# tahmidawal/Superresolution_for_PDEs

Hardware: AMD Instinct MI355X
Metric: 20->40 SR training samples/sec at batch 1024 per GPU (fwd+MSE bwd+clip+AdamW) (higher is better)
Workload: dtype f32 (h3: fp32 products from power-of-two-scaled 2-piece fp16 splits on fp16 MFMA, fp32 accumulate); 1 GPU; UNet 20->40 train step, fp32, batch 1024/GPU, 40x40; global_batch=1024, per_gpu_batch=1024, hw=40x40, parallelism=dp1

## Files before the change

### superresolution_for_pdes_amd/csrc/pointwise.hip

```cpp
#include "bn_reduce.h"

namespace srpde {

__global__ void nchw_to_nhwc_kernel(const float* __restrict__ x, float* __restrict__ out, int N, int Cin, int HW,
                                    int Cpad) {
  const long long total = (long long)N * HW;
  for (long long e = blockIdx.x * (long long)blockDim.x + threadIdx.x; e < total;
       e += (long long)gridDim.x * blockDim.x) {
    const long long n = e / HW;
    const int p = (int)(e - n * HW);
    float* o = out + e * Cpad;
    for (int c = 0; c < Cpad; ++c) o[c] = c < Cin ? x[(n * Cin + c) * HW + p] : 0.f;
  }
}

__global__ void nhwc_to_nchw_kernel(const float* __restrict__ x, int ldx, float* __restrict__ out, int N, int C,
                                    int HW) {
  const long long total = (long long)N * C * HW;
  for (long long e = blockIdx.x * (long long)blockDim.x + threadIdx.x; e < total;
       e += (long long)gridDim.x * blockDim.x) {
    const long long nc = e / HW;
    const int p = (int)(e - nc * HW);
    const long long n = nc / C;
    const int c = (int)(nc - n * C);
// ... 522 lines not shown
  }
  __syncthreads();
  for (int j = threadIdx.x; j < C; j += blockDim.x) m[(long long)n * C + j] = ms[j];
  for (int r = threadIdx.x; r < Cr; r += blockDim.x) {
    float a = b1[r];
    for (int c = 0; c < C; ++c) a += w1[r * C + c] * ms[c];
    a = fmaxf(a, 0.f);
    hs[r] = a;
    h[(long long)n * Cr + r] = a;
  }
  __syncthreads();
  for (int c = threadIdx.x; c < C; c += blockDim.x) {
    float a = b2[c];
    for (int r = 0; r < Cr; ++r) a += w2[c * Cr + r] * hs[r];
    ca[(long long)n * C + c] = 1.f / (1.f + expf(-a));
  }
}

__global__ __launch_bounds__(256) void att_spatial_fwd_kernel(const float* __restrict__ g, int ldg, long long P,
                                                              int G, const float* __restrict__ wg,
                                                              const float* __restrict__ bg, float* __restrict__ sa) {
  const int sub = threadIdx.x & 7;
  for (long long p = (blockIdx.x * (long long)blockDim.x + threadIdx.x) >> 3; p < P;
       p += ((long long)gridDim.x * blockDim.x) >> 3) {
    float acc = 0.f;
    const float* row = g + p * ldg;
    for (int c = sub * 4; c < G; c += 32) {
      const float4 v = ld4(row + c);
      const float4 w = ld4(wg + c);
      acc += dot4(v, w);
    }
    acc += __shfl_xor(acc, 1, 64);
    acc += __shfl_xor(acc, 2, 64);
    acc += __shfl_xor(acc, 4, 64);
    if (sub == 0) sa[p] = 1.f / (1.f + expf(-(acc + bg[0])));
  }
}

__global__ void att_apply_kernel(const float* __restrict__ x, int ldx, const float* __restrict__ ca,
                                 const float* __restrict__ sa, float* __restrict__ out, int ldo, long long P, int HW,
                                 int C) {
  const int C4 = C >> 2;
  const long long total = P * C4;
  for (long long e = blockIdx.x * (long long)blockDim.x + threadIdx.x; e < total;
       e += (long long)gridDim.x * blockDim.x) {
    const long long p = e / C4;
    const int c = (int)(e - p * C4) * 4;
    const long long n = p / HW;
    const float4 v = ld4(x + p * ldx + c);
    const float4 a = ld4(ca + n * C + c);
    const float s = sa[p];
    float4 o;
    o.x = (v.x * a.x) * s; o.y = (v.y * a.y) * s; o.z = (v.z * a.z) * s; o.w = (v.w * a.w) * s;
    *reinterpret_cast<float4*>(out + p * ldo + c) = o;
  }
}

__global__ __launch_bounds__(256) void att_bwd_pixel_kernel(const float* __restrict__ dout, int lddo,
                                                            const float* __restrict__ x, int ldx,
                                                            const float* __restrict__ ca,
                                                            const float* __restrict__ sa, long long P, int HW, int C,
                                                            float* __restrict__ dsa_pre) {
  const int sub = threadIdx.x & 7;
  for (long long p = (blockIdx.x * (long long)blockDim.x + threadIdx.x) >> 3; p < P;
       p += ((long long)gridDim.x * blockDim.x) >> 3) {
    const long long n = p / HW;
    float acc = 0.f;
    for (int c = sub * 4; c < C; c += 32) {
      const float4 d = ld4(dout + p * lddo + c);
      const float4 v = ld4(x + p * ldx + c);
      const float4 a = ld4(ca + n * C + c);
      acc += d.x * (v.x * a.x) + d.y * (v.y * a.y) + d.z * (v.z * a.z) + d.w * (v.w * a.w);
    }
    acc += __shfl_xor(acc, 1, 64);
    acc += __shfl_xor(acc, 2, 64);
    acc += __shfl_xor(acc, 4, 64);
    if (sub == 0) {
      const float s = sa[p];
      dsa_pre[p] = acc * (1.f - s) * s;
    }
  }
}

__global__ __launch_bounds__(256) void att_bwd_channel_kernel(
    const float* __restrict__ dout, int lddo, const float* __restrict__ x, int ldx, const float* __restrict__ sa,
    int HW, int C, int Cr, const float* __restrict__ w1, const float* __restrict__ w2, const float* __restrict__ m,
    const float* __restrict__ h, const float* __restrict__ ca, float* __restrict__ dm,
    float* __restrict__ dw1_rows, float* __restrict__ db1_rows, float* __restrict__ dw2_rows,
    float* __restrict__ db2_rows) {
  extern __shared__ float sh[];
  const int n = blockIdx.x, C4 = C >> 2;
  const int c4 = threadIdx.x % C4, r0 = threadIdx.x / C4, rs = blockDim.x / C4;
  const int active = C4 * rs;
  float4 s = zero4();
  if ((int)threadIdx.x < active) {
    const long long pb = (long long)n * HW;
    for (int p = r0; p < HW; p += rs) {
      const float4 d = ld4(dout + (pb + p) * lddo + c4 * 4);
      const float4 v = ld4(x + (pb + p) * ldx + c4 * 4);
      const float q = sa[pb + p];
      s.x += (d.x * q) * v.x; s.y += (d.y * q) * v.y; s.z += (d.z * q) * v.z; s.w += (d.w * q) * v.w;
    }
  }
  float4* red = reinterpret_cast<float4*>(sh);
  red[threadIdx.x] = s;
  __syncthreads();
  float* dpre = sh + 4 * 256;
  float* dh = dpre + C;
  if ((int)threadIdx.x < C4) {
    const float4 t = rowsum4(red, C4, rs, threadIdx.x);
    const int c = threadIdx.x * 4;
    const float tv[4] = {t.x, t.y, t.z, t.w};
#pragma unroll
    for (int k = 0; k < 4; ++k) {
      const float a = ca[(long long)n * C + c + k];
      dpre[c + k] = tv[k] * (1.f - a) * a;
    }
  }
  __syncthreads();
  for (int c = threadIdx.x; c < C; c += blockDim.x) db2_rows[(long long)n * C + c] = dpre[c];
  for (int r = threadIdx.x; r < Cr; r += blockDim.x) {
    float a = 0.f;
    for (int c = 0; c < C; ++c) a += w2[c * Cr + r] * dpre[c];
    a = h[(long long)n * Cr + r] > 0.f ? a : 0.f;
    dh[r] = a;
    db1_rows[(long long)n * Cr + r] = a;
  }
  __syncthreads();
  for (int c = threadIdx.x; c < C; c += blockDim.x) {
    float a = 0.f;
    for (int r = 0; r < Cr; ++r) a += w1[r * C + c] * dh[r];
    dm[(long long)n * C + c] = a / (float)HW;
  }
}

__global__ __launch_bounds__(256) void att_bwd_sample_kernel(
    const float* __restrict__ dout, int lddo, const float* __restrict__ x, int ldx, const float* __restrict__ sa,
    int HW, int C, int Cr, const float* __restrict__ w1, const float* __restrict__ w2, const float* __restrict__ m,
    const float* __restrict__ h, const float* __restrict__ ca, float* __restrict__ dm, float* __restrict__ dw1_rows,
    float* __restrict__ db1_rows, float* __restrict__ dw2_rows, float* __restrict__ db2_rows,
    float* __restrict__ dsa_pre) {
  extern __shared__ float sh[];
  const int n = blockIdx.x, C4 = C >> 2;
  const int c4 = threadIdx.x % C4, r0 = threadIdx.x / C4, rs = blockDim.x / C4;
  float4 s = zero4();
  {
    const float4 a = ld4(ca + (long long)n * C + c4 * 4);
    const long long pb = (long long)n * HW;
    for (int p = r0; p < HW; p += rs) {
      const float4 d = ld4(dout + (pb + p) * lddo + c4 * 4);
      const float4 v = ld4(x + (pb + p) * ldx + c4 * 4);
      const float q = sa[pb + p];
      s.x += (d.x * q) * v.x; s.y += (d.y * q) * v.y; s.z += (d.z * q) * v.z; s.w += (d.w * q) * v.w;
      float dot = d.x * (v.x * a.x) + d.y * (v.y * a.y) + d.z * (v.z * a.z) + d.w * (v.w * a.w);
      for (int o = C4 >> 1; o > 0; o >>= 1) dot += __shfl_xor(dot, o, 64);
      if (c4 == 0) dsa_pre[pb + p] = dot * (1.f - q) * q;
    }
  }
  float4* red = reinterpret_cast<float4*>(sh);
  red[threadIdx.x] = s;
  __syncthreads();
  float* dpre = sh + 4 * 256;
  float* dh = dpre + C;
  if ((int)threadIdx.x < C4) {
    const float4 t = rowsum4(red, C4, rs, threadIdx.x);
    const int c = threadIdx.x * 4;
    const float tv[4] = {t.x, t.y, t.z, t.w};
#pragma unroll
    for (int k = 0; k < 4; ++k) {
      const float a = ca[(long long)n * C + c + k];
      dpre[c + k] = tv[k] * (1.f - a) * a;
    }
  }
  __syncthreads();
  for (int c = threadIdx.x; c < C; c += blockDim.x) db2_rows[(long long)n * C + c] = dpre[c];
  for (int r = threadIdx.x; r < Cr; r += blockDim.x) {
    float a = 0.f;
    for (int c = 0; c < C; ++c) a += w2[c * Cr + r] * dpre[c];
    a = h[(long long)n * Cr + r] > 0.f ? a : 0.f;
    dh[r] = a;
    db1_rows[(long long)n * Cr + r] = a;
  }
  __syncthreads();
  for (int c = threadIdx.x; c < C; c += blockDim.x) {
    float a = 0.f;
    for (int r = 0; r < Cr; ++r) a += w1[r * C + c] * dh[r];
    dm[(long long)n * C + c] = a / (float)HW;
  }
}

__global__ void att_bwd_dx_kernel(const float* __restrict__ dout, int lddo, const float* __restrict__ ca,
                                  const float* __restrict__ sa, const float* __restrict__ dm, float* __restrict__ dx,
                                  int lddx, long long P, int HW, int C, int accumulate) {
  const int C4 = C >> 2;
  const long long total = P * C4;
  for (long long e = blockIdx.x * (long long)blockDim.x + threadIdx.x; e < total;
       e += (long long)gridDim.x * blockDim.x) {
    const long long p = e / C4;
    const int c = (int)(e - p * C4) * 4;
    const long long n = p / HW;
    const float4 d = ld4(dout + p * lddo + c);
    const float4 a = ld4(ca + n * C + c);
    const float4 g = ld4(dm + n * C + c);
    const float s = sa[p];
    float4 o = gate_dx4(d, s, a, g);
    float* dst = dx + p * lddx + c;
    if (accumulate) o = add4(o, ld4(dst));
    st4(dst, o);
  }
}

__global__ void att_bwd_gating_kernel(const float* __restrict__ dsa_pre, const float* __restrict__ wg,
                                      float* __restrict__ dg, int lddg, long long P, int G, int accumulate) {
  const int G4 = G >> 2;
  const long long total = P * G4;
  for (long long e = blockIdx.x * (long long)blockDim.x + threadIdx.x; e < total;
       e += (long long)gridDim.x * blockDim.x) {
    const long long p = e / G4;
    const int c = (int)(e - p * G4) * 4;
    const float s = dsa_pre[p];
    const float4 w = ld4(wg + c);
    float4 o = scale4(s, w);
    float* dst = dg + p * lddg + c;
    if (accumulate) o = add4(o, ld4(dst));
    st4(dst, o);
  }
}

__global__ __launch_bounds__(256) void weighted_colsum_kernel(const float* __restrict__ v, int ldv,
                                                              const float* __restrict__ s, long long P, int C,
                                                              int rows_per_blk, float2* __restrict__ part) {
  extern __shared__ float4 red4[];
  const int C4 = C >> 2;
  const int c4 = threadIdx.x % C4, r0 = threadIdx.x / C4, rs = blockDim.x / C4;
  const int active = C4 * rs;
  float4 acc = zero4();
  float sacc = 0.f;
  const long long pb = (long long)blockIdx.x * rows_per_blk;
  const long long pe = min(P, pb + rows_per_blk);
  if ((int)threadIdx.x < active) {
    auto row = [&](const float4& a, float w) {
      acc.x += a.x * w; acc.y += a.y * w; acc.z += a.z * w; acc.w += a.w * w;
      if (c4 == 0) sacc += w;
    };
    long long p = pb + r0;
    for (; p + 3 * rs < pe; p += 4 * rs) {
      float4 a[4];
      float w[4];
#pragma unroll
      for (int u = 0; u < 4; ++u) {
        a[u] = ld4(v + (p + u * rs) * ldv + c4 * 4);
        w[u] = s[p + u * rs];
      }
#pragma unroll
      for (int u = 0; u < 4; ++u) row(a[u], w[u]);
    }
    for (; p < pe; p += rs) row(ld4(v + p * ldv + c4 * 4), s[p]);
  }
  red4[threadIdx.x] = acc;
  red4[256 + threadIdx.x] = make_float4(sacc, 0.f, 0.f, 0.f);
  __syncthreads();
  if ((int)threadIdx.x < C4) {
    float4 t = zero4();
    float ts = 0.f;
    for (int r = 0; r < rs; ++r) {
      const float4 a = red4[r * C4 + threadIdx.x];
      t.x += a.x; t.y += a.y; t.z += a.z; t.w += a.w;
      if (threadIdx.x == 0) ts += red4[256 + r * C4].x;
    }
    float2* o = part + (size_t)blockIdx.x * (C + 1);
    const int c = threadIdx.x * 4;
    o[c] = make_float2(t.x, 0.f); o[c + 1] = make_float2(t.y, 0.f);
    o[c + 2] = make_float2(t.z, 0.f); o[c + 3] = make_float2(t.w, 0.f);
    if (threadIdx.x == 0) o[C] = make_float2(ts, 0.f);
  }
}

__global__ __launch_bounds__(1024) void outer_sum_kernel(const float* __restrict__ a, int la,
                                                         const float* __restrict__ b, int lb, int n,
                                                         float* __restrict__ out) {
  __shared__ double red[16][64];
  const int i = blockIdx.x, jl = threadIdx.x & 63, grp = threadIdx.x >> 6;
  const int j = blockIdx.y * 64 + jl;
  double s = 0.0;
  if (j < lb) {
    int k = grp;
    for (; k + 7 * 16 < n; k += 8 * 16) {
      float av[8], bv[8];
#pragma unroll
      for (int u = 0; u < 8; ++u) {
        av[u] = a ? a[(long long)(k + 16 * u) * la + i] : 1.f;
        bv[u] = b ? b[(long long)(k + 16 * u) * lb + j] : 1.f;
      }
#pragma unroll
      for (int u = 0; u < 8; ++u) s += (double)av[u] * (double)bv[u];
    }
    for (; k < n; k += 16) {
      const double av = a ? (double)a[(long long)k * la + i] : 1.0;
      const double bv = b ? (double)b[(long long)k * lb + j] : 1.0;
      s += av * bv;
    }
  }
  red[grp][jl] = s;
  __syncthreads();
  if (grp == 0 && j < lb) {
    double t = 0.0;
    for (int g = 0; g < 16; ++g) t += red[g][jl];
    out[(long long)i * lb + j] = (float)t;
  }
}

__global__ void rowsum_kernel(const float* __restrict__ rows, int n, int len, float* __restrict__ out, int stride_in,
                              int accumulate) {
  const int j = blockIdx.x * blockDim.x + threadIdx.x;
  if (j >= len) return;
  double s = 0.0;
  for (int k = 0; k < n; ++k) s += rows[(long long)k * stride_in + j];
  out[j] = accumulate ? out[j] + (float)s : (float)s;
}

__global__ void partsum_kernel(const float2* __restrict__ part, int nblk, int len, float* __restrict__ out) {
  const int j = blockIdx.x;
  __shared__ double a[256];
  double s = 0.0;
  for (int k = threadIdx.x; k < nblk; k += 256) s += part[(size_t)k * len + j].x;
  a[threadIdx.x] = s;
  __syncthreads();
  for (int t = 128; t > 0; t >>= 1) {
    if ((int)threadIdx.x < t) a[threadIdx.x] += a[threadIdx.x + t];
    __syncthreads();
  }
  if (threadIdx.x == 0) out[j] = (float)a[0];
}

__global__ void head_fwd_kernel(const float* __restrict__ z, int ldz, int C, const float* __restrict__ wf,
                                const float* __restrict__ bf, const float* __restrict__ xin, int xin_c, int HW,
                                long long P, float* __restrict__ out) {
  for (long long p = blockIdx.x * (long long)blockDim.x + threadIdx.x; p < P; p += (long long)gridDim.x * blockDim.x) {
    float acc = 0.f;
    for (int c = 0; c < C; c += 4) {
      const float4 v = ld4(z + p * ldz + c);
      acc += v.x * wf[c] + v.y * wf[c + 1] + v.z * wf[c + 2] + v.w * wf[c + 3];
    }
    const long long n = p / HW;
    const int q = (int)(p - n * HW);
    out[p] = (acc + bf[0]) + xin[(n * xin_c) * HW + q];
  }
}

__global__ void head_bwd_dz_kernel(const float* __restrict__ dout, const float* __restrict__ wf, int C,
                                   float* __restrict__ dz, int lddz, long long P) {
  const int C4 = C >> 2;
  const long long total = P * C4;
  for (long long e = blockIdx.x * (long long)blockDim.x + threadIdx.x; e < total;
       e += (long long)gridDim.x * blockDim.x) {
    const long long p = e / C4;
    const int c = (int)(e - p * C4) * 4;
    const float d = dout[p];
    *reinterpret_cast<float4*>(dz + p * lddz + c) = make_float4(d * wf[c], d * wf[c + 1], d * wf[c + 2], d * wf[c + 3]);
  }
}

__global__ __launch_bounds__(256) void mse_partial_kernel(const float* __restrict__ y, const float* __restrict__ t,
                                                          long long n, double* __restrict__ part) {
  __shared__ double red[256];
  double s = 0.0;
  for (long long i = blockIdx.x * (long long)blockDim.x + threadIdx.x; i < n; i += (long long)gridDim.x * blockDim.x) {
    const float d = y[i] - t[i];
    s += (double)(d * d);
  }
  red[threadIdx.x] = s;
  __syncthreads();
  for (int k = 128; k > 0; k >>= 1) {
    if ((int)threadIdx.x < k) red[threadIdx.x] += red[threadIdx.x + k];
    __syncthreads();
  }
  if (threadIdx.x == 0) part[blockIdx.x] = red[0];
}

__global__ void mse_final_kernel(const double* __restrict__ part, int nblk, long long n, float* __restrict__ loss) {
  __shared__ double red[256];
  double s = 0.0;
  for (int k = threadIdx.x; k < nblk; k += 256) s += part[k];
  red[threadIdx.x] = s;
  __syncthreads();
  for (int k = 128; k > 0; k >>= 1) {
    if ((int)threadIdx.x < k) red[threadIdx.x] += red[threadIdx.x + k];
    __syncthreads();
  }
  if (threadIdx.x == 0) loss[0] = (float)(red[0] / (double)n);
}

// ... 64 lines not shown
                         int w, int c, int accumulate, hipStream_t stream) {
  SRPDE_CHECK_ARG(x && dout && dx && c % 4 == 0 && h % 2 == 0 && w % 2 == 0, "srpde_maxpool2x2_bwd: bad args");
  launch_px_or_grid_stride(
      (long long)n * (h / 2) * (w / 2), c,
      [&](dim3 g, dim3 b, unsigned npix) {
        hipLaunchKernelGGL(maxpool2_bwd_px_kernel, g, b, 0, stream, x, ldx, dout, lddo, dx, lddx, npix, h, w, accumulate);
      },
      [&](dim3 g) {
        hipLaunchKernelGGL(maxpool2_bwd_kernel, g, dim3(256), 0, stream, x, ldx, dout, lddo, dx, lddx, n, h, w, c,
                           accumulate);
      });
  SRPDE_LAUNCH_CHECK("srpde_maxpool2x2_bwd");
  return 0;
}

int srpde_pde_dataset_assemble(const float* u_coarse, const float* u_fine, const float* theta_fine,
                               const float* f_fine, const float* stats, int theta_constant, int n, int hc, int wc,
                               int hf, int wf, float* inputs, float* targets, hipStream_t stream) {
  SRPDE_CHECK_ARG(u_coarse && u_fine && theta_fine && f_fine && stats && inputs && targets,
                  "srpde_pde_dataset_assemble: null");
  SRPDE_CHECK_ARG(n >= 0 && hc >= 1 && wc >= 1 && hf >= hc && wf >= wc, "srpde_pde_dataset_assemble: bad shape");
  if (n == 0) return 0;
  hipLaunchKernelGGL(pde_dataset_kernel, dim3(grid_for((long long)n * hf * wf)), dim3(256), 0, stream, u_coarse,
                     u_fine, theta_fine, f_fine, stats, theta_constant, n, hc, wc, hf, wf, inputs, targets);
  SRPDE_LAUNCH_CHECK("srpde_pde_dataset_assemble");
  return 0;
}

int srpde_upsample_bilinear_fwd(const float* x, int ldx, float* out, int ldo, int n, int h, int w, int ho, int wo,
                                int c, hipStream_t stream) {
  SRPDE_CHECK_ARG(x && out && c > 0, "srpde_upsample_bilinear_fwd: bad args");
  if (c % 4 != 0 || ldx % 4 != 0 || ldo % 4 != 0) {
    hipLaunchKernelGGL(upsample_fwd_scalar_kernel, dim3(grid_for((long long)n * ho * wo * c)), dim3(256), 0, stream,
                       x, ldx, out, ldo, n, h, w, ho, wo, c);
    SRPDE_LAUNCH_CHECK("srpde_upsample_bilinear_fwd");
    return 0;
  }
  launch_px_or_grid_stride(
      (long long)n * ho * wo, c,
      [&](dim3 g, dim3 b, unsigned npix) {
        hipLaunchKernelGGL(upsample_fwd_px_kernel, g, b, 0, stream, x, ldx, out, ldo, npix, h, w, ho, wo);
      },
      [&](dim3 g) {
        hipLaunchKernelGGL(upsample_fwd_kernel, g, dim3(256), 0, stream, x, ldx, out, ldo, n, h, w, ho, wo, c);
      });
  SRPDE_LAUNCH_CHECK("srpde_upsample_bilinear_fwd");
  return 0;
}

int srpde_upsample_bilinear_gate_fwd(const float* x, int ldx, float* out, int ldo, int n, int h, int w, int ho,
                                      int wo, int c, const float* wg, const float* bg, float* sa, hipStream_t stream) {
  SRPDE_CHECK_ARG(x && out && wg && bg && sa && ldx % 4 == 0 && ldo % 4 == 0 && c % 4 == 0 && c / 4 >= 1 &&
                      c / 4 <= 64 && ((c / 4) & (c / 4 - 1)) == 0,
                  "srpde_upsample_bilinear_gate_fwd: bad args (c / 4 a power of two <= 64)");
  dim3 g, b;
  SRPDE_CHECK_ARG(px_geometry((long long)n * ho * wo, c, &g, &b), "srpde_upsample_bilinear_gate_fwd: bad geometry");
  g.x = (g.x + UPX - 1) / UPX;
  hipLaunchKernelGGL(upsample_gate_fwd_px_kernel, g, b, 0, stream, x, ldx, out, ldo, (unsigned)(n * ho * wo), h, w,
                     ho, wo, wg, bg, sa);
  SRPDE_LAUNCH_CHECK("srpde_upsample_bilinear_gate_fwd");
  return 0;
}

size_t srpde_upsample_gate_sa_workspace_size(int n, int h, int w) { return (size_t)n * h * w * sizeof(float); }

int srpde_upsample_gate_sa(const float* x, int ldx, int n, int h, int w, int ho, int wo, int c, const float* wg,
                           const float* bg, float* sa, void* workspace, size_t ws_bytes, hipStream_t stream) {
  SRPDE_CHECK_ARG(x && wg && bg && sa && workspace && ldx % 4 == 0 && c % 4 == 0 && c / 4 >= 1 && c / 4 <= 64 &&
                      ((c / 4) & (c / 4 - 1)) == 0 && n > 0 && h > 0 && w > 0 && ho > 0 && wo > 0,
                  "srpde_upsample_gate_sa: bad args (c / 4 a power of two <= 64)");
  SRPDE_CHECK_ARG(ws_bytes >= srpde_upsample_gate_sa_workspace_size(n, h, w), "srpde_upsample_gate_sa: workspace");
  float* t = static_cast<float*>(workspace);
  dim3 g, b;
  SRPDE_CHECK_ARG(px_geometry((long long)n * h * w, c, &g, &b), "srpde_upsample_gate_sa: bad geometry");
  hipLaunchKernelGGL(gate_dot_px_kernel, g, b, 0, stream, x, ldx, (unsigned)(n * h * w), wg, t);
  SRPDE_LAUNCH_CHECK("srpde_upsample_gate_sa(dot)");
  const unsigned np = (unsigned)(n * ho * wo);
  hipLaunchKernelGGL(up_sigmoid_kernel, dim3((np + 255) / 256), dim3(256), 0, stream, t, sa, np, h, w, ho, wo, bg);
  SRPDE_LAUNCH_CHECK("srpde_upsample_gate_sa(up)");
  return 0;
}

static size_t att_lds_bytes(int c) { return (4 * 256 + c + c / 8) * sizeof(float); }

static void launch_att_channel(const float* x, int ldx, int n, int hw, int c, const float* w1, const float* b1,
                               const float* w2, const float* b2, float* m, float* hbuf, float* ca, hipStream_t stream) {
  hipLaunchKernelGGL(att_channel_fwd_kernel, dim3(n), dim3(256), att_lds_bytes(c), stream, x, ldx, hw, c, c / 8, w1, b1,
                     w2, b2, m, hbuf, ca);
}
static void launch_att_spatial(const float* g, int ldg, long long P, int gc, const float* wg, const float* bg, float* sa,
                               hipStream_t stream) {
  hipLaunchKernelGGL(att_spatial_fwd_kernel, dim3(grid_for(P * 8)), dim3(256), 0, stream, g, ldg, P, gc, wg, bg, sa);
}
static void launch_att_apply(const float* x, int ldx, const float* ca, const float* sa, float* out, int ldo, long long P,
                             int hw, int c, hipStream_t stream) {
  hipLaunchKernelGGL(att_apply_kernel, dim3(grid_for(P * (c / 4))), dim3(256), 0, stream, x, ldx, ca, sa, out, ldo, P,
                     hw, c);
}

int srpde_att_apply_fwd(const float* x, int ldx, int n, int hw, int c, const float* ca, const float* sa, float* out,
                        int ldo, hipStream_t stream) {
  SRPDE_CHECK_ARG(x && ca && sa && out && c % 4 == 0, "srpde_att_apply_fwd: bad args");
  launch_att_apply(x, ldx, ca, sa, out, ldo, (long long)n * hw, hw, c, stream);
  SRPDE_LAUNCH_CHECK("srpde_att_apply_fwd");
  return 0;
}

int srpde_upsample_bilinear_bwd_gated(const float* dout, int lddo, const float* dsa, const float* wg, float* dx,
                                      int lddx, int n, int h, int w, int ho, int wo, int c, int accumulate,
                                      hipStream_t stream) {
  SRPDE_CHECK_ARG(dout && dsa && wg && dx && c % 4 == 0 && lddo % 4 == 0 && lddx % 4 == 0 && ho >= h && wo >= w,
                  "srpde_upsample_bilinear_bwd_gated: bad args");
  SRPDE_CHECK_ARG(upsample_gather_ok(h, ho) && upsample_gather_ok(w, wo),
                  "srpde_upsample_bilinear_bwd_gated: upsampling ratio above 4 (%dx%d -> %dx%d)", h, w, ho, wo);
  if (upsample_rows_ok(h, w, ho, wo, c, lddo, lddx)) {
    launch_upsample_bwd_rows<true>(dout, lddo, dx, lddx, n, h, w, ho, wo, c, accumulate, dsa, wg, stream);
    SRPDE_LAUNCH_CHECK("srpde_upsample_bilinear_bwd_gated");
    return 0;
  }
  dim3 g, b;
  SRPDE_CHECK_ARG(px_geometry((long long)n * h * w, c, &g, &b),
                  "srpde_upsample_bilinear_bwd_gated: needs c / 4 a power of two <= 256 (c=%d)", c);
  hipLaunchKernelGGL(upsample_bwd_px_kernel, g, b, 0, stream, dout, lddo, dx, lddx, (unsigned)(n * h * w), h, w, ho,
                     wo, accumulate, dsa, wg);
  SRPDE_LAUNCH_CHECK("srpde_upsample_bilinear_bwd_gated");
  return 0;
}

int srpde_upsample_bwd_bn_supported(int h, int w, int ho, int wo, int c, int lddo, int lddx) {
  return upsample_gather_ok(h, ho) && upsample_gather_ok(w, wo) && upsample_rows_ok(h, w, ho, wo, c, lddo, lddx) ? 1
                                                                                                               : 0;
}

int srpde_upsample_bilinear_bwd_gated_bn(const float* dout, int lddo, const float* dsa, const float* wg, float* dx,
                                         int lddx, int n, int h, int w, int ho, int wo, int c, const float* y, int ldy,
                                         const float* mean, const float* invstd, const float* gamma,
                                         const float* beta, int flags, void* part, float* da_max,
                                         hipStream_t stream) {
  SRPDE_CHECK_ARG(dout && dsa && wg && dx && y && mean && invstd && gamma && beta && part && da_max && ldy % 4 == 0 &&
                      aligned16(y) && aligned16(dx) && aligned16(dout),
                  "srpde_upsample_bilinear_bwd_gated_bn: null argument / alignment");
  SRPDE_CHECK_ARG(ho >= h && wo >= w && srpde_upsample_bwd_bn_supported(h, w, ho, wo, c, lddo, lddx),
                  "srpde_upsample_bilinear_bwd_gated_bn: shape outside the row-blocked kernel "
                  "(srpde_upsample_bwd_bn_supported)");
  const UpBnArgs bn{y, ldy, mean, invstd, gamma, beta, flags & SRPDE_BN_RELU, static_cast<float2*>(part), da_max};
  launch_upsample_bwd_rows<true>(dout, lddo, dx, lddx, n, h, w, ho, wo, c, 0, dsa, wg, stream, &bn);
  SRPDE_LAUNCH_CHECK("srpde_upsample_bilinear_bwd_gated_bn");
  return 0;
}

int srpde_upsample_bilinear_bwd(const float* dout, int lddo, float* dx, int lddx, int n, int h, int w, int ho,
                                int wo, int c, int accumulate, hipStream_t stream) {
  SRPDE_CHECK_ARG(dout && dx && c % 4 == 0 && ho >= h && wo >= w, "srpde_upsample_bilinear_bwd: bad args");
  SRPDE_CHECK_ARG(upsample_gather_ok(h, ho) && upsample_gather_ok(w, wo),
                  "srpde_upsample_bilinear_bwd: upsampling ratio above 4 (%dx%d -> %dx%d)", h, w, ho, wo);
  if (upsample_rows_ok(h, w, ho, wo, c, lddo, lddx)) {
    launch_upsample_bwd_rows<false>(dout, lddo, dx, lddx, n, h, w, ho, wo, c, accumulate, nullptr, nullptr, stream);
    SRPDE_LAUNCH_CHECK("srpde_upsample_bilinear_bwd");
    return 0;
  }
  launch_px_or_grid_stride(
      (long long)n * h * w, c,
      [&](dim3 g, dim3 b, unsigned npix) {
        hipLaunchKernelGGL(upsample_bwd_px_kernel, g, b, 0, stream, dout, lddo, dx, lddx, npix, h, w, ho, wo, accumulate);
      },
      [&](dim3 g) {
        hipLaunchKernelGGL(upsample_bwd_kernel, g, dim3(256), 0, stream, dout, lddo, dx, lddx, n, h, w, ho, wo, c,
                           accumulate);
      });
  SRPDE_LAUNCH_CHECK("srpde_upsample_bilinear_bwd");
  return 0;
}

int srpde_att_channel_fwd(const float* x, int ldx, int n, int hw, int c, const float* w1, const float* b1,
                          const float* w2, const float* b2, float* m, float* hbuf, float* ca, hipStream_t stream) {
  SRPDE_CHECK_ARG(x && w1 && b1 && w2 && b2 && m && hbuf && ca, "srpde_att_channel_fwd: null");
  SRPDE_CHECK_ARG(c % 32 == 0 && c <= 1024, "srpde_att_channel_fwd: channel count");
  launch_att_channel(x, ldx, n, hw, c, w1, b1, w2, b2, m, hbuf, ca, stream);
  SRPDE_LAUNCH_CHECK("srpde_att_channel_fwd");
  return 0;
}

int srpde_att_gate_fwd(const float* x, int ldx, const float* g, int ldg, int n, int hw, int c, int gc,
                       const float* ca, const float* wg, const float* bg, float* sa, float* out, int ldo,
                       hipStream_t stream) {
  SRPDE_CHECK_ARG(x && g && ca && wg && bg && sa && out, "srpde_att_gate_fwd: null");
  SRPDE_CHECK_ARG(c % 32 == 0 && gc % 4 == 0 && c <= 1024, "srpde_att_gate_fwd: channel counts");
  const long long P = (long long)n * hw;
  launch_att_spatial(g, ldg, P, gc, wg, bg, sa, stream);
  SRPDE_LAUNCH_CHECK("srpde_att_gate_fwd(spatial)");
  launch_att_apply(x, ldx, ca, sa, out, ldo, P, hw, c, stream);
  SRPDE_LAUNCH_CHECK("srpde_att_gate_fwd(apply)");
  return 0;
}

int srpde_att_fwd(const float* x, int ldx, const float* g, int ldg, int n, int hw, int c, int gc, const float* w1,
                  const float* b1, const float* w2, const float* b2, const float* wg, const float* bg, float* m,
                  float* hbuf, float* ca, float* sa, float* out, int ldo, hipStream_t stream) {
  SRPDE_CHECK_ARG(x && g && w1 && b1 && w2 && b2 && wg && bg && m && hbuf && ca && sa && out,
                  "srpde_att_fwd: null");
  SRPDE_CHECK_ARG(c % 32 == 0 && gc % 4 == 0 && c <= 1024, "srpde_att_fwd: channel counts");
  launch_att_channel(x, ldx, n, hw, c, w1, b1, w2, b2, m, hbuf, ca, stream);
  SRPDE_LAUNCH_CHECK("srpde_att_fwd(channel)");
  const long long P = (long long)n * hw;
  launch_att_spatial(g, ldg, P, gc, wg, bg, sa, stream);
  SRPDE_LAUNCH_CHECK("srpde_att_fwd(spatial)");
  launch_att_apply(x, ldx, ca, sa, out, ldo, P, hw, c, stream);
  SRPDE_LAUNCH_CHECK("srpde_att_fwd(apply)");
  return 0;
}

size_t srpde_att_bwd_workspace_size(int n, int hw, int c, int gc) {
  if (!att_bwd_counts_ok(c, gc)) return 0;
  const long long P = (long long)n * hw;
  const int cr = c / 8;
  int rpb;
  const int nb = colsum_blocks(P, gc, &rpb);
  size_t f = (size_t)P
             + (size_t)n * c
             + (size_t)n * cr * c * 2
             + (size_t)n * (cr + c)
             + (size_t)nb * (gc + 1) * 2;
  return f * sizeof(float) + 256;
}

int srpde_att_bwd(const float* dout, int lddo, const float* x, int ldx, const float* g, int ldg, int n, int hw,
                  int c, int gc, const float* w1, const float* w2, const float* wg, const float* m, const float* hbuf,
                  const float* ca, const float* sa, float* dx, int lddx, int dx_accumulate, float* dg, int lddg,
                  int dg_accumulate, float* dw1, float* db1, float* dw2, float* db2, float* dwg, float* dbg,
                  void* workspace, size_t ws_bytes, hipStream_t stream) {
  SRPDE_CHECK_ARG(dout && x && g && workspace, "srpde_att_bwd: null");
  SRPDE_CHECK_ARG(att_bwd_counts_ok(c, gc), "srpde_att_bwd: channel counts (c %% 32, gc %% 4, both <= 1024)");
  if (ws_bytes < srpde_att_bwd_workspace_size(n, hw, c, gc)) {
    set_error("srpde_att_bwd: workspace too small");
    return kErrWorkspace;
  }
  const long long P = (long long)n * hw;
  const int cr = c / 8;
  float* dsa = static_cast<float*>(workspace);
  float* dm = dsa + P;
  float* dw1r = dm + (size_t)n * c;
  float* dw2r = dw1r + (size_t)n * cr * c;
  float* db1r = dw2r + (size_t)n * cr * c;
  float* db2r = db1r + (size_t)n * cr;
  float2* part = reinterpret_cast<float2*>(db2r + (size_t)n * c + 2);
  part = reinterpret_cast<float2*>((reinterpret_cast<uintptr_t>(part) + 15) & ~uintptr_t(15));

  const size_t lds = att_lds_bytes(c);
  if (c == 64 || c == 128 || c == 256) {
    hipLaunchKernelGGL(att_bwd_sample_kernel, dim3(n), dim3(256), lds, stream, dout, lddo, x, ldx, sa, hw, c, cr, w1,
                       w2, m, hbuf, ca, dm, dw1r, db1r, dw2r, db2r, dsa);
    SRPDE_LAUNCH_CHECK("srpde_att_bwd(sample)");
  } else {
    hipLaunchKernelGGL(att_bwd_pixel_kernel, dim3(grid_for(P * 8)), dim3(256), 0, stream, dout, lddo, x, ldx, ca,
                       sa, P, hw, c, dsa);
    SRPDE_LAUNCH_CHECK("srpde_att_bwd(pixel)");
    hipLaunchKernelGGL(att_bwd_channel_kernel, dim3(n), dim3(256), lds, stream, dout, lddo, x, ldx, sa, hw, c, cr,
                       w1, w2, m, hbuf, ca, dm, dw1r, db1r, dw2r, db2r);
    SRPDE_LAUNCH_CHECK("srpde_att_bwd(channel)");
  }
  if (dx != nullptr) {
    hipLaunchKernelGGL(att_bwd_dx_kernel, dim3(grid_for(P * (c / 4))), dim3(256), 0, stream, dout, lddo, ca, sa, dm,
                       dx, lddx, P, hw, c, dx_accumulate);
    SRPDE_LAUNCH_CHECK("srpde_att_bwd(dx)");
  }
  if (dg != nullptr) {
    hipLaunchKernelGGL(att_bwd_gating_kernel, dim3(grid_for(P * (gc / 4))), dim3(256), 0, stream, dsa, wg, dg, lddg,
                       P, gc, dg_accumulate);
    SRPDE_LAUNCH_CHECK("srpde_att_bwd(gating)");
  }
  if (dw1 == nullptr) return 0;
  return srpde_att_bwd_params(g, ldg, n, hw, c, gc, m, hbuf, dw1, db1, dw2, db2, dwg, dbg, workspace, ws_bytes,
                              stream);
}

__global__ __launch_bounds__(256) void upsample_t_scalar_kernel(const float* __restrict__ dsa, float* __restrict__ st,
                                                                int n, int h, int w, int ho, int wo) {
  const long long q = (long long)blockIdx.x * blockDim.x + threadIdx.x;
  if (q >= (long long)n * h * w) return;
  const int ix = (int)(q % w), iy = (int)((q / w) % h), nn = (int)(q / ((long long)w * h));
  int ylo, yhi, xlo, xhi;
  cand_range(iy, h, ho, &ylo, &yhi);
  cand_range(ix, w, wo, &xlo, &xhi);
  const float* base = dsa + (size_t)nn * ho * wo;
  float s = 0.f;
  for (int oy = ylo; oy <= yhi; ++oy) {
    bool hy;
    const float wy = cand_weight(oy, iy, h, ho, &hy);
    if (!hy) continue;
    float r = 0.f;
    for (int ox = xlo; ox <= xhi; ++ox) {
      bool hx;
      const float wx = cand_weight(ox, ix, w, wo, &hx);
      if (hx) r += wx * base[(size_t)oy * wo + ox];
    }
    s += wy * r;
  }
  st[q] = s;
}

static void att_params_outer(int n, int c, const float* m, const float* hbuf, const float* db1r, const float* db2r,
                             float* dw1, float* db1, float* dw2, float* db2, hipStream_t stream) {
  const int cr = c / 8;
  hipLaunchKernelGGL(outer_sum_kernel, dim3(cr, ceil_div(c, 64)), dim3(1024), 0, stream, db1r, cr, m, c, n, dw1);
  hipLaunchKernelGGL(outer_sum_kernel, dim3(c, ceil_div(cr, 64)), dim3(1024), 0, stream, db2r, c, hbuf, cr, n, dw2);
  hipLaunchKernelGGL(outer_sum_kernel, dim3(1, ceil_div(cr, 64)), dim3(1024), 0, stream, (const float*)nullptr, 1,
                     db1r, cr, n, db1);
  hipLaunchKernelGGL(outer_sum_kernel, dim3(1, ceil_div(c, 64)), dim3(1024), 0, stream, (const float*)nullptr, 1,
                     db2r, c, n, db2);
}

int srpde_att_bwd_params_lowres(const float* d, int ldd, int n, int h, int w, int ho, int wo, int c, int gc,
                                const float* m, const float* hbuf, float* dw1, float* db1, float* dw2, float* db2,
                                float* dwg, float* dbg, void* workspace, size_t ws_bytes, hipStream_t stream) {
  SRPDE_CHECK_ARG(d && m && hbuf && dw1 && db1 && dw2 && db2 && dwg && dbg && workspace && ldd % 4 == 0 && ho >= h &&
                      wo >= w,
                  "srpde_att_bwd_params_lowres: bad args");
  SRPDE_CHECK_ARG(att_bwd_counts_ok(c, gc),
                  "srpde_att_bwd_params_lowres: channel counts (c %% 32, gc %% 4, both <= 1024)");
  const int hw = ho * wo;
  if (ws_bytes < srpde_att_bwd_workspace_size(n, hw, c, gc)) {
    set_error("srpde_att_bwd_params_lowres: workspace too small");
    return kErrWorkspace;
  }
  const long long P = (long long)n * hw, Plo = (long long)n * h * w;
  const int cr = c / 8;
  float* dsa = static_cast<float*>(workspace);
  float* dm = dsa + P;
  float* dw1r = dm + (size_t)n * c;
  float* dw2r = dw1r + (size_t)n * cr * c;
  float* db1r = dw2r + (size_t)n * cr * c;
  float* db2r = db1r + (size_t)n * cr;
  float2* part = reinterpret_cast<float2*>(db2r + (size_t)n * c + 2);
  part = reinterpret_cast<float2*>((reinterpret_cast<uintptr_t>(part) + 15) & ~uintptr_t(15));
  SRPDE_CHECK_ARG(Plo <= 2LL * n * cr * c, "srpde_att_bwd_params_lowres: low-res field larger than its scratch");
  float* st = dw1r;
  att_params_outer(n, c, m, hbuf, db1r, db2r, dw1, db1, dw2, db2, stream);
  SRPDE_LAUNCH_CHECK("srpde_att_bwd_params_lowres(rowsum)");
  hipLaunchKernelGGL(upsample_t_scalar_kernel, dim3((unsigned)((Plo + 255) / 256)), dim3(256), 0, stream, dsa, st, n, h,
                     w, ho, wo);
  SRPDE_LAUNCH_CHECK("srpde_att_bwd_params_lowres(transpose)");
  int rpb;
  const int nb = colsum_blocks(Plo, gc, &rpb);
  hipLaunchKernelGGL(weighted_colsum_kernel, dim3(nb), dim3(256), 2 * 256 * sizeof(float4), stream, d, ldd, st, Plo,
                     gc, rpb, part);
  SRPDE_LAUNCH_CHECK("srpde_att_bwd_params_lowres(colsum)");
  hipLaunchKernelGGL(partsum_kernel, dim3(gc), dim3(256), 0, stream, part, nb, gc + 1, dwg);
  hipLaunchKernelGGL(partsum_kernel, dim3(1), dim3(256), 0, stream, part + gc, nb, gc + 1, dbg);
  SRPDE_LAUNCH_CHECK("srpde_att_bwd_params_lowres(partsum)");
  return 0;
}

int srpde_att_bwd_params(const float* g, int ldg, int n, int hw, int c, int gc, const float* m, const float* hbuf,
                         float* dw1, float* db1, float* dw2, float* db2, float* dwg, float* dbg, void* workspace,
                         size_t ws_bytes, hipStream_t stream) {
  SRPDE_CHECK_ARG(g && m && hbuf && dw1 && db1 && dw2 && db2 && dwg && dbg && workspace,
                  "srpde_att_bwd_params: null");
  SRPDE_CHECK_ARG(att_bwd_counts_ok(c, gc), "srpde_att_bwd_params: channel counts (c %% 32, gc %% 4, both <= 1024)");
  if (ws_bytes < srpde_att_bwd_workspace_size(n, hw, c, gc)) {
    set_error("srpde_att_bwd_params: workspace too small");
    return kErrWorkspace;
  }
  const long long P = (long long)n * hw;
  const int cr = c / 8;
  float* dsa = static_cast<float*>(workspace);
  float* dm = dsa + P;
  float* dw1r = dm + (size_t)n * c;
  float* dw2r = dw1r + (size_t)n * cr * c;
  float* db1r = dw2r + (size_t)n * cr * c;
  float* db2r = db1r + (size_t)n * cr;
  float2* part = reinterpret_cast<float2*>(db2r + (size_t)n * c + 2);
  part = reinterpret_cast<float2*>((reinterpret_cast<uintptr_t>(part) + 15) & ~uintptr_t(15));
  (void)dw1r; (void)dw2r; (void)cr;
  att_params_outer(n, c, m, hbuf, db1r, db2r, dw1, db1, dw2, db2, stream);
  SRPDE_LAUNCH_CHECK("srpde_att_bwd(rowsum)");
  int rpb;
  const int nb = colsum_blocks(P, gc, &rpb);
  hipLaunchKernelGGL(weighted_colsum_kernel, dim3(nb), dim3(256), 2 * 256 * sizeof(float4), stream, g, ldg, dsa, P,
                     gc, rpb, part);
  SRPDE_LAUNCH_CHECK("srpde_att_bwd(colsum)");
  hipLaunchKernelGGL(partsum_kernel, dim3(gc), dim3(256), 0, stream, part, nb, gc + 1, dwg);
  hipLaunchKernelGGL(partsum_kernel, dim3(1), dim3(256), 0, stream, part + gc, nb, gc + 1, dbg);
  SRPDE_LAUNCH_CHECK("srpde_att_bwd(partsum)");
  return 0;
}

int srpde_head_fwd(const float* z, int ldz, int c, const float* wf, const float* bf, const float* xin, int xin_c,
                   int n, int hw, float* out, hipStream_t stream) {
  SRPDE_CHECK_ARG(z && wf && bf && xin && out && c % 4 == 0, "srpde_head_fwd: bad args");
  const long long P = (long long)n * hw;
  hipLaunchKernelGGL(head_fwd_kernel, dim3(grid_for(P)), dim3(256), 0, stream, z, ldz, c, wf, bf, xin, xin_c, hw, P,
                     out);
  SRPDE_LAUNCH_CHECK("srpde_head_fwd");
  return 0;
}

size_t srpde_head_bwd_workspace_size(int n, int hw, int c) {
  if (!colsum_ok(c)) return 0;
  int rpb;
  const int nb = colsum_blocks((long long)n * hw, c, &rpb);
  return (size_t)nb * (c + 1) * sizeof(float2);
}

int srpde_head_bwd(const float* dout, const float* z, int ldz, int c, const float* wf, int n, int hw, float* dz,
                   int lddz, float* dwf, float* dbf, void* workspace, size_t ws_bytes, hipStream_t stream) {
  SRPDE_CHECK_ARG(dout && z && wf && dz && dwf && dbf && workspace, "srpde_head_bwd: bad args");
  SRPDE_CHECK_ARG(colsum_ok(c), "srpde_head_bwd: channel count (c %% 4, 4 <= c <= 1024)");
  if (ws_bytes < srpde_head_bwd_workspace_size(n, hw, c)) {
    set_error("srpde_head_bwd: workspace too small");
    return kErrWorkspace;
  }
  const long long P = (long long)n * hw;
  hipLaunchKernelGGL(head_bwd_dz_kernel, dim3(grid_for(P * (c / 4))), dim3(256), 0, stream, dout, wf, c, dz, lddz, P);
  SRPDE_LAUNCH_CHECK("srpde_head_bwd(dz)");
  int rpb;
  const int nb = colsum_blocks(P, c, &rpb);
  float2* part = static_cast<float2*>(workspace);
  hipLaunchKernelGGL(weighted_colsum_kernel, dim3(nb), dim3(256), 2 * 256 * sizeof(float4), stream, z, ldz, dout, P,
                     c, rpb, part);
  hipLaunchKernelGGL(partsum_kernel, dim3(c), dim3(256), 0, stream, part, nb, c + 1, dwf);
  hipLaunchKernelGGL(partsum_kernel, dim3(1), dim3(256), 0, stream, part + c, nb, c + 1, dbf);
  SRPDE_LAUNCH_CHECK("srpde_head_bwd(reduce)");
  return 0;
}

size_t srpde_mse_workspace_size(void) { return 1024 * sizeof(double); }

int srpde_mse_fwd(const float* y, const float* t, long long n, float* loss, void* workspace, size_t ws_bytes,
                  hipStream_t stream) {
  SRPDE_CHECK_ARG(y && t && loss && workspace && ws_bytes >= 1024 * sizeof(double), "srpde_mse_fwd: bad args");
  const int nb = (int)std::min<long long>(1024, std::max<long long>(1, (n + 255) / 256));
  hipLaunchKernelGGL(mse_partial_kernel, dim3(nb), dim3(256), 0, stream, y, t, n, static_cast<double*>(workspace));
  hipLaunchKernelGGL(mse_final_kernel, dim3(1), dim3(256), 0, stream, static_cast<const double*>(workspace), nb, n,
                     loss);
  SRPDE_LAUNCH_CHECK("srpde_mse_fwd");
  return 0;
}

int srpde_mse_bwd(const float* y, const float* t, long long n, const float* gout, float* dy, hipStream_t stream) {
  SRPDE_CHECK_ARG(y && t && dy, "srpde_mse_bwd: bad args");
  hipLaunchKernelGGL(mse_bwd_kernel, dim3(grid_for(n)), dim3(256), 0, stream, y, t, n, gout, dy);
  SRPDE_LAUNCH_CHECK("srpde_mse_bwd");
  return 0;
}

}
```

Before: 37680 samples/s.

## Tile attention MLP weight-gradient reduction and stage w2 in LDS

Replaces the four outer_sum launches for the attention MLP weight and bias gradients with one tiled kernel. It stages per-sample dh, h, dpre and m slices in LDS and accumulates all four gradients in double, split across sample slices, with a second kernel summing the partials. The backward per-sample kernels now stage w2 into shared memory for the dpre->dh matvec and unroll the pixel loop by four to issue more loads at once. The cost is more LDS per block, which may reduce occupancy, plus an extra partial-sum pass through scratch memory.

Measured after the change: 37810 samples/s (median of 6 runs). Within noise of the previous version (+0.3%).

```diff
diff --git a/superresolution_for_pdes_amd/csrc/pointwise.hip b/superresolution_for_pdes_amd/csrc/pointwise.hip
--- a/superresolution_for_pdes_amd/csrc/pointwise.hip
+++ b/superresolution_for_pdes_amd/csrc/pointwise.hip
@@ -628,6 +628,45 @@
   }
 }
 
+constexpr int kAttW2Stage = 8192;
+
+__device__ __forceinline__ void stage_floats(float* dst, const float* __restrict__ src, int count) {
+  if ((reinterpret_cast<uintptr_t>(src) & 15u) == 0) {
+    for (int i = threadIdx.x * 4; i < count; i += blockDim.x * 4) st4(dst + i, ld4(src + i));
+  } else {
+    for (int i = threadIdx.x; i < count; i += blockDim.x) dst[i] = src[i];
+  }
+}
+
+__device__ __forceinline__ void att_mlp_bwd_tail(const float* dpre, float* dh, float* w2s, int n, int HW, int C, int Cr,
+                                                 const float* __restrict__ w1, const float* __restrict__ w2,
+                                                 const float* __restrict__ h, float* __restrict__ dm,
+                                                 float* __restrict__ db1_rows, float* __restrict__ db2_rows) {
+  for (int c = threadIdx.x; c < C; c += blockDim.x) db2_rows[(long long)n * C + c] = dpre[c];
+  const int r = threadIdx.x;
+  const int rows = min(C, kAttW2Stage / Cr);
+  float a = 0.f;
+  for (int c0 = 0; c0 < C; c0 += rows) {
+    const int nc = min(rows, C - c0);
+    if (c0 > 0) __syncthreads();
+    stage_floats(w2s, w2 + (long long)c0 * Cr, nc * Cr);
+    __syncthreads();
+    if (r < Cr)
+      for (int c = 0; c < nc; ++c) a += w2s[c * Cr + r] * dpre[c0 + c];
+  }
+  if (r < Cr) {
+    a = h[(long long)n * Cr + r] > 0.f ? a : 0.f;
+    dh[r] = a;
+    db1_rows[(long long)n * Cr + r] = a;
+  }
+  __syncthreads();
+  for (int c = threadIdx.x; c < C; c += blockDim.x) {
+    float a = 0.f;
+    for (int r = 0; r < Cr; ++r) a += w1[r * C + c] * dh[r];
+    dm[(long long)n * C + c] = a / (float)HW;
+  }
+}
+
 __global__ __launch_bounds__(256) void att_bwd_channel_kernel(
     const float* __restrict__ dout, int lddo, const float* __restrict__ x, int ldx, const float* __restrict__ sa,
     int HW, int C, int Cr, const float* __restrict__ w1, const float* __restrict__ w2, const float* __restrict__ m,
@@ -664,20 +703,7 @@
     }
   }
   __syncthreads();
-  for (int c = threadIdx.x; c < C; c += blockDim.x) db2_rows[(long long)n * C + c] = dpre[c];
-  for (int r = threadIdx.x; r < Cr; r += blockDim.x) {
-    float a = 0.f;
-    for (int c = 0; c < C; ++c) a += w2[c * Cr + r] * dpre[c];
-    a = h[(long long)n * Cr + r] > 0.f ? a : 0.f;
-    dh[r] = a;
-    db1_rows[(long long)n * Cr + r] = a;
-  }
-  __syncthreads();
-  for (int c = threadIdx.x; c < C; c += blockDim.x) {
-    float a = 0.f;
-    for (int r = 0; r < Cr; ++r) a += w1[r * C + c] * dh[r];
-    dm[(long long)n * C + c] = a / (float)HW;
-  }
+  att_mlp_bwd_tail(dpre, dh, dh + Cr, n, HW, C, Cr, w1, w2, h, dm, db1_rows, db2_rows);
 }
 
 __global__ __launch_bounds__(256) void att_bwd_sample_kernel(
@@ -693,15 +719,27 @@
   {
     const float4 a = ld4(ca + (long long)n * C + c4 * 4);
     const long long pb = (long long)n * HW;
-    for (int p = r0; p < HW; p += rs) {
-      const float4 d = ld4(dout + (pb + p) * lddo + c4 * 4);
-      const float4 v = ld4(x + (pb + p) * ldx + c4 * 4);
-      const float q = sa[pb + p];
+    auto pixel = [&](int p, const float4& d, const float4& v, float q) {
       s.x += (d.x * q) * v.x; s.y += (d.y * q) * v.y; s.z += (d.z * q) * v.z; s.w += (d.w * q) * v.w;
       float dot = d.x * (v.x * a.x) + d.y * (v.y * a.y) + d.z * (v.z * a.z) + d.w * (v.w * a.w);
       for (int o = C4 >> 1; o > 0; o >>= 1) dot += __shfl_xor(dot, o, 64);
       if (c4 == 0) dsa_pre[pb + p] = dot * (1.f - q) * q;
-    }
+    };
+    int p = r0;
+    for (; p + 3 * rs < HW; p += 4 * rs) {
+      float4 d[4], v[4];
+      float q[4];
+#pragma unroll
+      for (int u = 0; u < 4; ++u) {
+        d[u] = ld4(dout + (pb + p + u * rs) * lddo + c4 * 4);
+        v[u] = ld4(x + (pb + p + u * rs) * ldx + c4 * 4);
+        q[u] = sa[pb + p + u * rs];
+      }
+#pragma unroll
+      for (int u = 0; u < 4; ++u) pixel(p + u * rs, d[u], v[u], q[u]);
+    }
+    for (; p < HW; p += rs)
+      pixel(p, ld4(dout + (pb + p) * lddo + c4 * 4), ld4(x + (pb + p) * ldx + c4 * 4), sa[pb + p]);
   }
   float4* red = reinterpret_cast<float4*>(sh);
   red[threadIdx.x] = s;
@@ -719,20 +757,7 @@
     }
   }
   __syncthreads();
-  for (int c = threadIdx.x; c < C; c += blockDim.x) db2_rows[(long long)n * C + c] = dpre[c];
-  for (int r = threadIdx.x; r < Cr; r += blockDim.x) {
-    float a = 0.f;
-    for (int c = 0; c < C; ++c) a += w2[c * Cr + r] * dpre[c];
-    a = h[(long long)n * Cr + r] > 0.f ? a : 0.f;
-    dh[r] = a;
-    db1_rows[(long long)n * Cr + r] = a;
-  }
-  __syncthreads();
-  for (int c = threadIdx.x; c < C; c += blockDim.x) {
-    float a = 0.f;
-    for (int r = 0; r < Cr; ++r) a += w1[r * C + c] * dh[r];
-    dm[(long long)n * C + c] = a / (float)HW;
-  }
+  att_mlp_bwd_tail(dpre, dh, dh + Cr, n, HW, C, Cr, w1, w2, h, dm, db1_rows, db2_rows);
 }
 
 __global__ void att_bwd_dx_kernel(const float* __restrict__ dout, int lddo, const float* __restrict__ ca,
@@ -822,38 +847,125 @@
   }
 }
 
-__global__ __launch_bounds__(1024) void outer_sum_kernel(const float* __restrict__ a, int la,
-                                                         const float* __restrict__ b, int lb, int n,
-                                                         float* __restrict__ out) {
-  __shared__ double red[16][64];
-  const int i = blockIdx.x, jl = threadIdx.x & 63, grp = threadIdx.x >> 6;
-  const int j = blockIdx.y * 64 + jl;
+constexpr int kAttParSamples = 32;
+constexpr int kAttParCols = 32;
+
+template <int NR>
+__global__ __launch_bounds__(256) void att_params_kernel(const float* __restrict__ dh, const float* __restrict__ dpre,
+                                                         const float* __restrict__ m, const float* __restrict__ h,
+                                                         int n, int C, int Cr, int per_slice,
+                                                         double* __restrict__ part, float* __restrict__ dw1,
+                                                         float* __restrict__ db1, float* __restrict__ dw2,
+                                                         float* __restrict__ db2) {
+  constexpr int SB = kAttParSamples, CB = kAttParCols;
+  extern __shared__ float sh[];
+  float* sdh = sh;
+  float* shh = sdh + SB * Cr;
+  float* sdp = shh + SB * Cr;
+  float* sm = sdp + SB * CB;
+  const int t = threadIdx.x, j = t & (CB - 1), rg = t / CB;
+  const int col0 = blockIdx.y * CB;
+  const int kb = blockIdx.x * per_slice, ke = min(n, kb + per_slice);
+  int r1[NR], c2[NR], r2[NR];
+  double a1[NR], a2[NR], s1[NR], s2 = 0.0;
+#pragma unroll
+  for (int i = 0; i < NR; ++i) {
+    r1[i] = min(rg + 8 * i, Cr - 1);
+    const int f = min(t + 256 * i, CB * Cr - 1);
+    c2[i] = f / Cr;
+    r2[i] = f - c2[i] * Cr;
+    a1[i] = a2[i] = s1[i] = 0.0;
+  }
+  const bool al = ((reinterpret_cast<uintptr_t>(dh) | reinterpret_cast<uintptr_t>(dpre) |
+                    reinterpret_cast<uintptr_t>(m) | reinterpret_cast<uintptr_t>(h)) & 15u) == 0;
+  for (int k0 = kb; k0 < ke; k0 += SB) {
+    const int ns = min(SB, ke - k0), nq = ns * Cr;
+    if (k0 > kb) __syncthreads();
+    if (al) {
+      const int ks = t >> 3, q = (t & 7) * 4;
+      float4 p4 = zero4(), m4 = zero4();
+      if (ks < ns) {
+        p4 = ld4(dpre + (long long)(k0 + ks) * C + col0 + q);
+        m4 = ld4(m + (long long)(k0 + ks) * C + col0 + q);
+      }
+      for (int i = t * 4; i < nq; i += 1024) {
+        const float4 x0 = ld4(dh + (long long)k0 * Cr + i);
+        const float4 x1 = ld4(h + (long long)k0 * Cr + i);
+        st4(sdh + i, x0);
+        st4(shh + i, x1);
+      }
+      if (ks < ns) {
+        st4(sdp + ks * CB + q, p4);
+        st4(sm + ks * CB + q, m4);
+      }
+    } else {
+      for (int i = t; i < ns * CB; i += 256) {
+        const long long g = (long long)(k0 + i / CB) * C + col0 + (i & (CB - 1));
+        sdp[i] = dpre[g];
+        sm[i] = m[g];
+      }
+      for (int i = t; i < nq; i += 256) {
+        sdh[i] = dh[(long long)k0 * Cr + i];
+        shh[i] = h[(long long)k0 * Cr + i];
+      }
+    }
+    __syncthreads();
+    for (int k = 0; k < ns; ++k) {
+      const double mv = (double)sm[k * CB + j], pv = (double)sdp[k * CB + j];
+      s2 += pv;
+#pragma unroll
+      for (int i = 0; i < NR; ++i) {
+        const double dv = (double)sdh[k * Cr + r1[i]];
+        a1[i] += dv * mv;
+        s1[i] += dv;
+        a2[i] += (double)sdp[k * CB + c2[i]] * (double)shh[k * Cr + r2[i]];
+      }
+    }
+  }
+  const int W = Cr * C;
+  double* P = part ? part + (size_t)blockIdx.x * (2 * W + Cr + C) : nullptr;
+#pragma unroll
+  for (int i = 0; i < NR; ++i) {
+    const int r = rg + 8 * i, f = t + 256 * i;
+    if (r < Cr) {
+      const int e = r * C + col0 + j;
+      if (P) P[e] = a1[i];
+      else dw1[e] = (float)a1[i];
+      if (j == 0 && blockIdx.y == 0) {
+        if (P) P[2 * W + r] = s1[i];
+        else db1[r] = (float)s1[i];
+      }
+    }
+    if (f < CB * Cr) {
+      const int e = col0 * Cr + f;
+      if (P) P[W + e] = a2[i];
+      else dw2[e] = (float)a2[i];
+    }
+  }
+  if (rg == 0) {
+    if (P) P[2 * W + Cr + col0 + j] = s2;
+    else db2[col0 + j] = (float)s2;
+  }
+}
+
+__global__ __launch_bounds__(256) void att_params_sum_kernel(const double* __restrict__ part, int slices, int C, int Cr,
+                                                             float* __restrict__ dw1, float* __restrict__ db1,
+                                                             float* __restrict__ dw2, float* __restrict__ db2) {
+  const int W = Cr * C, E = 2 * W + Cr + C;
+  const int e = blockIdx.x * 256 + threadIdx.x;
+  if (e >= E) return;
   double s = 0.0;
-  if (j < lb) {
-    int k = grp;
-    for (; k + 7 * 16 < n; k += 8 * 16) {
-      float av[8], bv[8];
-#pragma unroll
-      for (int u = 0; u < 8; ++u) {
-        av[u] = a ? a[(long long)(k + 16 * u) * la + i] : 1.f;
-        bv[u] = b ? b[(long long)(k + 16 * u) * lb + j] : 1.f;
-      }
-#pragma unroll
-      for (int u = 0; u < 8; ++u) s += (double)av[u] * (double)bv[u];
-    }
-    for (; k < n; k += 16) {
-      const double av = a ? (double)a[(long long)k * la + i] : 1.0;
-      const double bv = b ? (double)b[(long long)k * lb + j] : 1.0;
-      s += av * bv;
-    }
-  }
-  red[grp][jl] = s;
-  __syncthreads();
-  if (grp == 0 && j < lb) {
-    double t = 0.0;
-    for (int g = 0; g < 16; ++g) t += red[g][jl];
-    out[(long long)i * lb + j] = (float)t;
-  }
+  int k = 0;
+  for (; k + 7 < slices; k += 8) {
+    double v[8];
+#pragma unroll
+    for (int u = 0; u < 8; ++u) v[u] = part[(size_t)(k + u) * E + e];
+#pragma unroll
+    for (int u = 0; u < 8; ++u) s += v[u];
+  }
+  for (; k < slices; ++k) s += part[(size_t)k * E + e];
+  float* o = e < W ? dw1 + e : e < 2 * W ? dw2 + (e - W) : e < 2 * W + Cr ? db1 + (e - 2 * W) : db2 + (e - 2 * W - Cr);
+  *o = (float)s;
 }
 
 __global__ void rowsum_kernel(const float* __restrict__ rows, int n, int len, float* __restrict__ out, int stride_in,
@@ -1084,6 +1196,9 @@
 }
 
 static size_t att_lds_bytes(int c) { return (4 * 256 + c + c / 8) * sizeof(float); }
+static size_t att_bwd_lds_bytes(int c) {
+  return att_lds_bytes(c) + (size_t)std::min(c * (c / 8), kAttW2Stage) * sizeof(float);
+}
 
 static void launch_att_channel(const float* x, int ldx, int n, int hw, int c, const float* w1, const float* b1,
                                const float* w2, const float* b2, float* m, float* hbuf, float* ca, hipStream_t stream) {
@@ -1248,7 +1363,7 @@
   float2* part = reinterpret_cast<float2*>(db2r + (size_t)n * c + 2);
   part = reinterpret_cast<float2*>((reinterpret_cast<uintptr_t>(part) + 15) & ~uintptr_t(15));
 
-  const size_t lds = att_lds_bytes(c);
+  const size_t lds = att_bwd_lds_bytes(c);
   if (c == 64 || c == 128 || c == 256) {
     hipLaunchKernelGGL(att_bwd_sample_kernel, dim3(n), dim3(256), lds, stream, dout, lddo, x, ldx, sa, hw, c, cr, w1,
                        w2, m, hbuf, ca, dm, dw1r, db1r, dw2r, db2r, dsa);
@@ -1302,14 +1417,35 @@
 }
 
 static void att_params_outer(int n, int c, const float* m, const float* hbuf, const float* db1r, const float* db2r,
-                             float* dw1, float* db1, float* dw2, float* db2, hipStream_t stream) {
+                             float* dw1, float* db1, float* dw2, float* db2, float* scratch, size_t scratch_floats,
+                             hipStream_t stream) {
   const int cr = c / 8;
-  hipLaunchKernelGGL(outer_sum_kernel, dim3(cr, ceil_div(c, 64)), dim3(1024), 0, stream, db1r, cr, m, c, n, dw1);
-  hipLaunchKernelGGL(outer_sum_kernel, dim3(c, ceil_div(cr, 64)), dim3(1024), 0, stream, db2r, c, hbuf, cr, n, dw2);
-  hipLaunchKernelGGL(outer_sum_kernel, dim3(1, ceil_div(cr, 64)), dim3(1024), 0, stream, (const float*)nullptr, 1,
-                     db1r, cr, n, db1);
-  hipLaunchKernelGGL(outer_sum_kernel, dim3(1, ceil_div(c, 64)), dim3(1024), 0, stream, (const float*)nullptr, 1,
-                     db2r, c, n, db2);
+  const size_t e = 2 * (size_t)cr * c + cr + c;
+  double* part = reinterpret_cast<double*>((reinterpret_cast<uintptr_t>(scratch) + 15) & ~uintptr_t(15));
+  const size_t room = std::min<size_t>(scratch_floats >= 4 ? (scratch_floats - 4) / (2 * e) : 0, 256);
+  int per = kAttParSamples, slices = ceil_div(n, per);
+  if (slices > 1 && room < 2) {
+    per = n;
+    slices = 1;
+  } else if ((size_t)slices > room && slices > 1) {
+    per = kAttParSamples * ceil_div(n, (long long)kAttParSamples * room);
+    slices = ceil_div(n, per);
+  }
+  if (slices == 1) part = nullptr;
+  const dim3 grid(slices, c / kAttParCols);
+  const size_t lds = (size_t)kAttParSamples * (2 * cr + 2 * kAttParCols) * sizeof(float);
+  auto go = [&](auto kernel) {
+    hipLaunchKernelGGL(kernel, grid, dim3(256), lds, stream, db1r, db2r, m, hbuf, n, c, cr, per, part, dw1, db1, dw2,
+                       db2);
+  };
+  if (cr <= 8) go(att_params_kernel<1>);
+  else if (cr <= 16) go(att_params_kernel<2>);
+  else if (cr <= 32) go(att_params_kernel<4>);
+  else if (cr <= 64) go(att_params_kernel<8>);
+  else go(att_params_kernel<16>);
+  if (part != nullptr)
+    hipLaunchKernelGGL(att_params_sum_kernel, dim3(ceil_div((long long)e, 256)), dim3(256), 0, stream, part, slices, c,
+                       cr, dw1, db1, dw2, db2);
 }
 
 int srpde_att_bwd_params_lowres(const float* d, int ldd, int n, int h, int w, int ho, int wo, int c, int gc,
@@ -1337,7 +1473,7 @@
   part = reinterpret_cast<float2*>((reinterpret_cast<uintptr_t>(part) + 15) & ~uintptr_t(15));
   SRPDE_CHECK_ARG(Plo <= 2LL * n * cr * c, "srpde_att_bwd_params_lowres: low-res field larger than its scratch");
   float* st = dw1r;
-  att_params_outer(n, c, m, hbuf, db1r, db2r, dw1, db1, dw2, db2, stream);
+  att_params_outer(n, c, m, hbuf, db1r, db2r, dw1, db1, dw2, db2, dw1r, 2 * (size_t)n * cr * c, stream);
   SRPDE_LAUNCH_CHECK("srpde_att_bwd_params_lowres(rowsum)");
   hipLaunchKernelGGL(upsample_t_scalar_kernel, dim3((unsigned)((Plo + 255) / 256)), dim3(256), 0, stream, dsa, st, n, h,
                      w, ho, wo);
@@ -1373,8 +1509,7 @@
   float* db2r = db1r + (size_t)n * cr;
   float2* part = reinterpret_cast<float2*>(db2r + (size_t)n * c + 2);
   part = reinterpret_cast<float2*>((reinterpret_cast<uintptr_t>(part) + 15) & ~uintptr_t(15));
-  (void)dw1r; (void)dw2r; (void)cr;
-  att_params_outer(n, c, m, hbuf, db1r, db2r, dw1, db1, dw2, db2, stream);
+  att_params_outer(n, c, m, hbuf, db1r, db2r, dw1, db1, dw2, db2, dw1r, 2 * (size_t)n * cr * c, stream);
   SRPDE_LAUNCH_CHECK("srpde_att_bwd(rowsum)");
   int rpb;
   const int nb = colsum_blocks(P, gc, &rpb);
```
